# lrm2017/Fastest_Image_Pattern_Matching

Hardware: AMD Instinct MI355X
Metric: template matches/sec + ms/search, 4024×3036 src ±180°; HBM GB/s vs roofline (higher is better)
Workload: dtype u8

## Files before the change

fastest_image_pattern_matching_amd/csrc/fpm_kernels.hip:

```cpp
#include <float.h>
#include <stdio.h>
#include <stdlib.h>
#include <limits.h>

#include <map>
#include <mutex>
#include <type_traits>
#include <utility>

#include "../../include/fpm.h"
#include "fpm_kernels.h"
#include "fpm_model.h"
#include "fpm_rrect.h"

static void ensure_lds_attr(const void* fn, size_t bytes) {
    if (bytes <= 65536) return;
    int dev = 0;
    (void)hipGetDevice(&dev);
    static std::mutex mu;
    static std::map<std::pair<int, const void*>, size_t> done;
    std::lock_guard<std::mutex> lock(mu);
    size_t& cur = done[std::make_pair(dev, fn)];
    if (bytes <= cur) return;
    (void)hipFuncSetAttribute(fn, hipFuncAttributeMaxDynamicSharedMemorySize, (int)bytes);
// ... 2191 lines not shown

__device__ __forceinline__ int mad24(int a, int b, int c) {
    int d;
    asm("v_mad_i32_i24 %0, %1, %2, %3" : "=v"(d) : "v"(a), "v"(b), "v"(c));
    return d;
}

__device__ __forceinline__ int ft_tap_interior(const uint8_t* FT, int off, int ftw, int X, int Y) {
    const uint32_t fx = X & (kInterTab - 1), fy = Y & (kInterTab - 1);
    const uint32_t* F = (const uint32_t*)FT;
    const int off1 = off + ftw;
    const uint32_t* q0 = F + (off >> 2);
    const uint32_t* q1 = F + (off1 >> 2);
    const uint32_t r0 = __builtin_amdgcn_alignbyte(q0[1], q0[0], (uint32_t)off);
    const uint32_t r1 = __builtin_amdgcn_alignbyte(q1[1], q1[0], (uint32_t)off1);
    const uint32_t wx = 32u + fx * 255u;
    const uint32_t h0 = __builtin_amdgcn_udot4(r0, wx, 0u, false), h1 = __builtin_amdgcn_udot4(r1, wx, 0u, false);
    return (int)((__umul24(32u - fy, h0) + __umul24(fy, h1) + 512u) >> 10);
}

__device__ __forceinline__ int ft_tap_bytes(const uint8_t* FT, int off, int ftw, int X, int Y) {
    const int fx = X & (kInterTab - 1), fy = Y & (kInterTab - 1);
    const uint8_t* p = FT + off;
    const int v0 = p[0], v1 = p[1], v2 = p[ftw], v3 = p[ftw + 1];
    const int h0 = 32 * v0 + __mul24(fx, v1 - v0), h1 = 32 * v2 + __mul24(fx, v3 - v2);
    return (32 * h0 + __mul24(fy, h1 - h0) + 512) >> 10;
}

typedef __attribute__((address_space(3))) const uint8_t fpm_lds_u8;
__device__ __forceinline__ uint32_t lds_offset_of(const uint8_t* p) { return (uint32_t)(size_t)(fpm_lds_u8*)p; }
__device__ __forceinline__ void lds_taps(uint32_t off, int ftw, int v[4]) {
    fpm_lds_u8* p = (fpm_lds_u8*)(size_t)off;
    fpm_lds_u8* q = (fpm_lds_u8*)(size_t)(off + ftw);
    v[0] = p[0]; v[1] = p[1]; v[2] = q[0]; v[3] = q[1];
}
__device__ __forceinline__ int bilerp24(const int v[4], int fx, int fy) {
    const int h0 = mad24(fx, v[1] - v[0], v[0] << 5), h1 = mad24(fx, v[3] - v[2], v[2] << 5);
    return mad24(fy, h1 - h0, (h0 << 5) + 512) >> 10;
}
typedef unsigned short fpm_u16x2v __attribute__((ext_vector_type(2)));
__device__ __forceinline__ uint32_t bilerp_row4(const int v[4][4], const int fx[4], const int fy[4]) {
    uint32_t r[4];
#pragma unroll
    for (int u = 0; u < 4; ++u) {
        const uint32_t a02 = __builtin_amdgcn_perm((uint32_t)v[u][2], (uint32_t)v[u][0], 0x0c040c00u);
        const uint32_t a13 = __builtin_amdgcn_perm((uint32_t)v[u][3], (uint32_t)v[u][1], 0x0c040c00u);
        const fpm_u16x2v d = __builtin_bit_cast(fpm_u16x2v, a13) - __builtin_bit_cast(fpm_u16x2v, a02);
        const fpm_u16x2v b = __builtin_bit_cast(fpm_u16x2v, a02) << (fpm_u16x2v)5;
        uint32_t h;
        asm("v_pk_mad_u16 %0, %1, %2, %3 op_sel_hi:[0,1,1]"
            : "=v"(h) : "v"(fx[u]), "v"(__builtin_bit_cast(uint32_t, d)), "v"(__builtin_bit_cast(uint32_t, b)));
        const uint32_t wy = (uint32_t)mad24(fy[u], 64 * 0x10000 - 64, 64 * 32);
        r[u] = __builtin_amdgcn_udot2(__builtin_bit_cast(fpm_u16x2v, h), __builtin_bit_cast(fpm_u16x2v, wy), 64u * 512u,
                                      false);
    }
    return __builtin_amdgcn_perm(r[1], r[0], 0x0c0c0602u) | __builtin_amdgcn_perm(r[3], r[2], 0x06020c0cu);
}
template <int PITCH>
__device__ __forceinline__ void lds_taps16(const uint32_t off[4], int v[4][4]) {
    asm volatile("ds_read_u8 %0, %16\n\tds_read_u8 %1, %16 offset:1\n\tds_read_u8 %2, %16 offset:%20\n\t"
                 "ds_read_u8 %3, %16 offset:%21\n\t"
                 "ds_read_u8 %4, %17\n\tds_read_u8 %5, %17 offset:1\n\tds_read_u8 %6, %17 offset:%20\n\t"
                 "ds_read_u8 %7, %17 offset:%21\n\t"
                 "ds_read_u8 %8, %18\n\tds_read_u8 %9, %18 offset:1\n\tds_read_u8 %10, %18 offset:%20\n\t"
                 "ds_read_u8 %11, %18 offset:%21\n\t"
                 "ds_read_u8 %12, %19\n\tds_read_u8 %13, %19 offset:1\n\tds_read_u8 %14, %19 offset:%20\n\t"
                 "ds_read_u8 %15, %19 offset:%21\n\t"
                 "s_waitcnt lgkmcnt(0)"
                 : "=&v"(v[0][0]), "=&v"(v[0][1]), "=&v"(v[0][2]), "=&v"(v[0][3]), "=&v"(v[1][0]), "=&v"(v[1][1]),
                   "=&v"(v[1][2]), "=&v"(v[1][3]), "=&v"(v[2][0]), "=&v"(v[2][1]), "=&v"(v[2][2]), "=&v"(v[2][3]),
                   "=&v"(v[3][0]), "=&v"(v[3][1]), "=&v"(v[3][2]), "=&v"(v[3][3])
                 : "v"(off[0]), "v"(off[1]), "v"(off[2]), "v"(off[3]), "i"(PITCH), "i"(PITCH + 1)
                 : "memory");
}

__device__ __forceinline__ int ft_tap_general(const uint8_t* FT, int ftw, int bxa, int by0, int W, int H, int X, int Y) {
    const int sx = sat_s16(X >> kInterBits), sy = sat_s16(Y >> kInterBits);
    const int fx = X & (kInterTab - 1), fy = Y & (kInterTab - 1);
    const uint8_t* p = FT + (sy - by0) * ftw + (sx - bxa);
    int v0, v1, v2, v3;
    if ((unsigned)sx < (unsigned)(W - 1) && (unsigned)sy < (unsigned)(H - 1)) {
        v0 = p[0]; v1 = p[1]; v2 = p[ftw]; v3 = p[ftw + 1];
    } else if (sx >= W || sx + 1 < 0 || sy >= H || sy + 1 < 0) {
        return 0;
    } else {
        const bool x0 = sx >= 0 && sx < W, x1 = sx + 1 >= 0 && sx + 1 < W;
        const bool y0 = sy >= 0 && sy < H, y1 = sy + 1 >= 0 && sy + 1 < H;
        v0 = x0 && y0 ? p[0] : 0;
        v1 = x1 && y0 ? p[1] : 0;
        v2 = x0 && y1 ? p[ftw] : 0;
        v3 = x1 && y1 ? p[ftw + 1] : 0;
    }
    const int h0 = 32 * v0 + fx * (v1 - v0), h1 = 32 * v2 + fx * (v3 - v2);
    return (32 * h0 + fy * (h1 - h0) + 512) >> 10;
}

__device__ __forceinline__ int roi_base(const RoiArgs& a) { return a.slot_base; }
__device__ __forceinline__ void roi_slot(const RoiArgs& a, int slot, int& id, int& jj) {
    const int ri = roi_base(a) + slot;
    const int li = ri / a.n3;
    jj = ri - li * a.n3;
    id = a.live[li];
}

__device__ __forceinline__ int roi_count(const RoiArgs& a) {
    int rois = *a.live_count * a.n3 - roi_base(a);
    return rois < 0 ? 0 : (rois > a.slot_cap ? a.slot_cap : rois);
}

__device__ __forceinline__ void wave_sync() {
    __builtin_amdgcn_fence(__ATOMIC_RELEASE, "wavefront");
    __builtin_amdgcn_wave_barrier();
    __builtin_amdgcn_fence(__ATOMIC_ACQUIRE, "wavefront");
}

template <int B>
__device__ __forceinline__ void stage_footprint(uint8_t* FT, int ftw, int wpr, int fth, const uint8_t* gsrc,
                                                size_t gpitch, int gx0, int gP, int lane) {
    const int c = lane & 15;
    if (c >= wpr) return;
    const int gx = gx0 + 4 * c;
    const bool inb = gx < gP;
    const uint8_t* gp = gsrc + 4 * c + (size_t)(lane >> 4) * gpitch;
    uint8_t* lp = FT + 4 * c + (lane >> 4) * ftw;
    const size_t gstep = 4 * gpitch;
    const int lstep = 4 * ftw;
    for (int r0 = lane >> 4; r0 < fth; r0 += 4 * B) {
        uint32_t v[B];
#pragma unroll
        for (int i = 0; i < B; ++i) v[i] = (inb && r0 + 4 * i < fth) ? *(const uint32_t*)(gp + i * gstep) : 0u;
#pragma unroll
        for (int i = 0; i < B; ++i)
            if (r0 + 4 * i < fth) *(uint32_t*)(lp + i * lstep) = v[i];
        gp += B * gstep;
        lp += B * lstep;
    }
}
typedef __attribute__((address_space(3))) void* fpm_lds_vp;
typedef __attribute__((address_space(1))) void* fpm_gbl_vp;
__device__ __forceinline__ void stage_footprint_dma(uint8_t* FT, int wpr, int fth, const uint8_t* gsrc,
                                                    size_t gpitch, int lane) {
    const int total = wpr * fth;
    int r = lane / wpr, c = lane - r * wpr;
    const int dr = 64 / wpr, dc = 64 - dr * wpr;
    for (int i0 = 0; i0 < total; i0 += 64) {
        if (i0 + lane < total)
            __builtin_amdgcn_global_load_lds((fpm_gbl_vp)(gsrc + (size_t)r * gpitch + 4 * c), (fpm_lds_vp)(FT + 4 * i0), 4, 0, 0);
        r += dr;
        c += dc;
        if (c >= wpr) { c -= wpr; ++r; }
    }
    asm volatile("s_waitcnt vmcnt(0)" ::: "memory");
}
__device__ __forceinline__ void stage_block16(uint8_t* dst, int dp, const uint8_t* src, size_t sp, int rows, int q16,
                                              int tid, int nthr) {
    const int total = rows * q16;
    int r = tid / q16, c = tid - (tid / q16) * q16;
    const int dr = nthr / q16, dc = nthr - dr * q16;
    for (int i0 = tid; i0 < total; i0 += 4 * nthr) {
        uint4 v[4];
        int rr[4], cc[4];
#pragma unroll
        for (int k = 0; k < 4; ++k) {
            rr[k] = r; cc[k] = c;
            v[k] = (i0 + k * nthr < total) ? *(const uint4*)(src + (size_t)r * sp + 16 * c) : make_uint4(0, 0, 0, 0);
            r += dr; c += dc;
            if (c >= q16) { c -= q16; ++r; }
        }
#pragma unroll
        for (int k = 0; k < 4; ++k)
            if (i0 + k * nthr < total) *(uint4*)(dst + (size_t)rr[k] * dp + 16 * cc[k]) = v[k];
    }
}
__device__ __forceinline__ void stage_block4(uint8_t* dst, int dp, const uint8_t* src, size_t sp, int rows, int wpr,
                                             int gx0, int gP, int tid, int nthr) {
    const int total = rows * wpr;
    int r = tid / wpr, c = tid - (tid / wpr) * wpr;
    const int dr = nthr / wpr, dc = nthr - dr * wpr;
    for (int i0 = tid; i0 < total; i0 += 8 * nthr) {
        uint32_t v[8];
        int rr[8], cc[8];
#pragma unroll
        for (int k = 0; k < 8; ++k) {
            rr[k] = r; cc[k] = c;
            v[k] = (i0 + k * nthr < total && gx0 + 4 * c < gP) ? *(const uint32_t*)(src + (size_t)r * sp + 4 * c) : 0u;
            r += dr; c += dc;
            if (c >= wpr) { c -= wpr; ++r; }
        }
#pragma unroll
        for (int k = 0; k < 8; ++k)
            if (i0 + k * nthr < total) *(uint32_t*)(dst + (size_t)rr[k] * dp + 4 * cc[k]) = v[k];
    }
}

constexpr int kPatchTw = 64, kPatchTh = 16;
constexpr int kPatchFtPitch = 76;
constexpr int kPatchFtRows = 72;

constexpr int kPatchTabWords = 2 * kPatchTw + 2 * kPatchTh;
constexpr int kPatchFtBytes = kPatchFtPitch * kPatchFtRows + 16;

struct PatchTile {
    int job;
    int x0, y0;
    int bxa, by0;
    bool in_lds;
    const uint8_t* img;
};

__device__ __forceinline__ PatchTile patch_tile_stage_at(const PatchArgs& a, int32_t* tab, uint8_t* FT, int tid, int p,
                                                         int tx, int ty) {
    int32_t* const ad = tab;
    int32_t* const bd = tab + kPatchTw;
    int32_t* const X0 = tab + 2 * kPatchTw;
    int32_t* const Y0 = X0 + kPatchTh;
    const int x0 = tx * kPatchTw, y0 = ty * kPatchTh;
    const PatchJob& j = a.jobs[p];
    if (tid < kPatchTw) {
        const int x = x0 + tid;
        ad[tid] = rint_i(j.M[0] * x * kAbScale);
        bd[tid] = rint_i(j.M[3] * x * kAbScale);
    } else if (tid < kPatchTw + kPatchTh) {
        const int y = y0 + tid - kPatchTw;
        X0[tid - kPatchTw] = rint_i((j.M[1] * y + j.M[2]) * kAbScale) + kRoundDelta;
        Y0[tid - kPatchTw] = rint_i((j.M[4] * y + j.M[5]) * kAbScale) + kRoundDelta;
    }
    __syncthreads();
    const int cx = (a.pw - x0 < kPatchTw ? a.pw - x0 : kPatchTw) - 1, cy = (a.ph - y0 < kPatchTh ? a.ph - y0 : kPatchTh) - 1;
    int bx0 = INT_MAX, bx1 = INT_MIN, by0 = INT_MAX, by1 = INT_MIN;
#pragma unroll
    for (int k = 0; k < 4; ++k) {
        const int c = (k & 1) ? cx : 0, r = (k & 2) ? cy : 0;
        const int sx = (X0[r] + ad[c]) >> kAbBits, sy = (Y0[r] + bd[c]) >> kAbBits;
        bx0 = sx < bx0 ? sx : bx0; bx1 = sx > bx1 ? sx : bx1;
        by0 = sy < by0 ? sy : by0; by1 = sy > by1 ? sy : by1;
    }
    bx0 -= 1; by0 -= 1; bx1 += 2; by1 += 2;
    const int bxa = bx0 & ~3;
    const int wpr = ((bx1 - bxa) >> 2) + 1;
    const int fth = by1 - by0 + 1;
    const bool fits = bx0 >= 0 && by0 >= 0 && bx1 < a.sw && by1 < a.sh && a.sw <= 32768 && a.sh <= 32768 &&
                      wpr <= kPatchFtPitch / 4 && fth <= kPatchFtRows;
    const bool in_lds = __builtin_amdgcn_readfirstlane((int)fits) != 0;
    const uint8_t* img = a.level0 + (size_t)j.src * a.img_stride;
    if (in_lds) {
        stage_block4(FT, kPatchFtPitch, img + (size_t)by0 * a.sp + bxa, (size_t)a.sp, fth, wpr, bxa, a.sp, tid, 256);
        __syncthreads();
    }
    return {p, x0, y0, bxa, by0, in_lds, img};
}

__device__ __forceinline__ PatchTile patch_tile_stage(const PatchArgs& a, int32_t* tab, uint8_t* FT, int tid) {
    const int b = xcd_remap(blockIdx.x, gridDim.x);
    const int tiles = a.tiles_x * a.tiles_y;
    const int p = b / tiles, t = b - p * tiles;
    const int ty = t / a.tiles_x, tx = t - ty * a.tiles_x;
    return patch_tile_stage_at(a, tab, FT, tid, p, tx, ty);
}

__device__ __forceinline__ uint32_t patch_sample4(const PatchArgs& a, const PatchTile& T, const int32_t* tab,
                                                  const uint8_t* FT, int r, int gx, int nu) {
    const int Xr = tab[2 * kPatchTw + r], Yr = tab[2 * kPatchTw + kPatchTh + r];
    const int4 A = *(const int4*)(tab + gx), B = *(const int4*)(tab + kPatchTw + gx);
    const int av[4] = {A.x, A.y, A.z, A.w}, bv[4] = {B.x, B.y, B.z, B.w};
    uint32_t word = 0;
#pragma unroll
    for (int u = 0; u < 4; ++u) {
        if (u >= nu) break;
        const int X = (Xr + av[u]) >> (kAbBits - kInterBits), Y = (Yr + bv[u]) >> (kAbBits - kInterBits);
        int v;
        if (T.in_lds)
            v = ft_tap_bytes(FT, ((Y >> kInterBits) - T.by0) * kPatchFtPitch + (X >> kInterBits) - T.bxa, kPatchFtPitch, X, Y);
        else
            v = warp_tap(T.img, a.sw, a.sh, a.sp, X, Y, 0);
        word |= (uint32_t)v << (8 * u);
    }
    return word;
}

__device__ __forceinline__ void patch_store4(uint8_t* d, uint32_t word, int nu, bool dword) {
    if (dword && nu == 4) {
        *(uint32_t*)d = word;
    } else {
        for (int u = 0; u < nu; ++u) d[u] = (uint8_t)(word >> (8 * u));
    }
}

__global__ __launch_bounds__(256) void k_patch_warp(const PatchArgs a) {
    __shared__ __attribute__((aligned(16))) int32_t tab[kPatchTabWords];
    __shared__ __attribute__((aligned(16))) uint8_t FT[kPatchFtBytes];
    const int tid = threadIdx.x;
    const PatchTile T = patch_tile_stage(a, tab, FT, tid);
    const int r = tid >> 4, gx = (tid & 15) * 4;
    const int x = T.x0 + gx, y = T.y0 + r;
    if (x >= a.pw || y >= a.ph) return;
    const int nu = a.pw - x < 4 ? a.pw - x : 4;
    const uint32_t word = patch_sample4(a, T, tab, FT, r, gx, nu);
    patch_store4(a.out + a.jobs[T.job].out_off + (size_t)y * a.row_stride + x, word, nu, a.dword != 0);
}

template <int CTRL, int ROWS, bool MAX>
__device__ __forceinline__ uint32_t dpp_fold(uint32_t v) {
    const uint32_t o = (uint32_t)__builtin_amdgcn_update_dpp(0, (int)v, CTRL, ROWS, 0xf, false);
    return MAX ? (o > v ? o : v) : v + o;
}
template <bool MAX>
__device__ __forceinline__ uint32_t wave_fold(uint32_t v) {
    v = dpp_fold<0xb1, 0xf, MAX>(v);
    v = dpp_fold<0x4e, 0xf, MAX>(v);
    v = dpp_fold<0x141, 0xf, MAX>(v);
    v = dpp_fold<0x140, 0xf, MAX>(v);
    v = dpp_fold<0x142, 0xa, MAX>(v);
    v = dpp_fold<0x143, 0xc, MAX>(v);
    return (uint32_t)__builtin_amdgcn_readlane((int)v, 63);
}

__device__ __forceinline__ void vote_box(unsigned long long mk, int u, int& cnt, int& cmin, int& cmax, int& rmin,
                                         int& rmax) {
    if (mk == 0) return;
    cnt += __popcll(mk);
    const uint32_t cols = (uint32_t)(mk | (mk >> 16) | (mk >> 32) | (mk >> 48)) & 0xffffu;
    const int lo = 4 * (__ffs(cols) - 1) + u, hi = 4 * (31 - __clz(cols)) + u;
    cmin = lo < cmin ? lo : cmin; cmax = hi > cmax ? hi : cmax;
    const int rlo = (__ffsll(mk) - 1) >> 4, rhi = (63 - __clzll(mk)) >> 4;
    rmin = rlo < rmin ? rlo : rmin; rmax = rhi > rmax ? rhi : rmax;
}
// ... 1803 lines not shown
            const uint32_t l0 = row[0] ^ 0x80808080u, l1 = row[1] ^ 0x80808080u;
            const int wr = tw >> 2;
            const uint32_t x0 = row[wr], x1 = row[wr + 1], x2 = row[wr + 2];
            const uint32_t e0 = __builtin_amdgcn_alignbyte(x1, x0, (uint32_t)tw) ^ 0x80808080u;
            const uint32_t e1 = __builtin_amdgcn_alignbyte(x2, x1, (uint32_t)tw) ^ 0x80808080u;
            s1 += (uint32_t)__builtin_amdgcn_mov_dpp((int)s1, 0xB1, 0xF, 0xF, false);
            s2 += (uint32_t)__builtin_amdgcn_mov_dpp((int)s2, 0xB1, 0xF, 0xF, false);
            s1 += (uint32_t)__builtin_amdgcn_mov_dpp((int)s1, 0x4E, 0xF, 0xF, false);
            s2 += (uint32_t)__builtin_amdgcn_mov_dpp((int)s2, 0x4E, 0xF, 0xF, false);
#pragma unroll
            for (int h = 0; h < 2; ++h) {
                const int dx = qq + 4 * h;
                if (dx < 7) {
                    const uint32_t ml0 = dx >= 4 ? 0xffffffffu : (1u << (8 * dx)) - 1u;
                    const uint32_t ml1 = dx <= 4 ? 0u : (1u << (8 * (dx - 4))) - 1u;
                    const uint32_t mr0 = dx >= 4 ? 0u : ~((1u << (8 * dx)) - 1u);
                    const uint32_t mr1 = dx <= 4 ? 0xffffu : dx == 5 ? 0xff00u : 0u;
                    const uint32_t a0 = l0 & ml0, a1 = l1 & ml1, b0 = e0 & mr0, b1 = e1 & mr1;
                    uint32_t q1 = __builtin_amdgcn_udot4(a0, 0x01010101u, 0u, false);
                    q1 = __builtin_amdgcn_udot4(a1, 0x01010101u, q1, false);
                    q1 = __builtin_amdgcn_udot4(b0, 0x01010101u, q1, false);
                    q1 = __builtin_amdgcn_udot4(b1, 0x01010101u, q1, false);
                    uint32_t q2 = __builtin_amdgcn_udot4(a0, a0, 0u, false);
                    q2 = __builtin_amdgcn_udot4(a1, a1, q2, false);
                    q2 = __builtin_amdgcn_udot4(b0, b0, q2, false);
                    q2 = __builtin_amdgcn_udot4(b1, b1, q2, false);
                    const uint32_t v1 = s1 - q1, v2 = s2 - q2;
                    wi[r * 7 + dx] = v1;
                    wq[r * 7 + dx] = v2;
                    if (MODE != 6) {
                        if (r < rb) { u1[h] = v1; u2[h] = v2; }
                        const uint32_t eo = (uint32_t)slot * (uint32_t)kRoiEdgeWords;
                        if (band == 0 && r < 6) {
                            const uint32_t o = eo + (uint32_t)(r * 7 + dx);
                            a.wedge[o] = v1;
                            a.wedge[o + 84u] = v2;
                        }
                        if (band == nband - 1 && r >= rb) {
                            const uint32_t o = eo + (uint32_t)((6 + r - rb) * 7 + dx);
                            a.wedge[o] = v1;
                            a.wedge[o + 84u] = v2;
                        }
                    }
                }
            }
        }
        if (RS == 1 && MODE != 7 && MODE != 6 && wv < 2) {
#pragma unroll
            for (int h = 0; h < 2; ++h) {
                uint32_t r1 = u1[h], lo = u2[h] & 0xffffu, hi = u2[h] >> 16;
#pragma unroll
                for (int m = 4; m <= 32; m <<= 1) {
                    r1 += (uint32_t)__shfl_xor((int)r1, m, 64);
                    lo += (uint32_t)__shfl_xor((int)lo, m, 64);
                    hi += (uint32_t)__shfl_xor((int)hi, m, 64);
                }
                if (lane < 4 && lane + 4 * h < 7) {
                    bt1[8 * wv + lane + 4 * h] = r1;
                    bt2[8 * wv + lane + 4 * h] = (uint64_t)lo + ((uint64_t)hi << 16);
                }
            }
        }
        __syncthreads();
        auto band_totals = [&]() {
            if (MODE == 6 || MODE == 7 || tid < 128 || tid >= 128 + 7) return;
            uint32_t dx = (uint32_t)(tid - 128);
            asm volatile("" : "+v"(dx));
            const bool two = rb > kMmaRows;
            const uint32_t s1 = bt1[dx] + (two ? bt1[8 + dx] : 0u);
            const uint64_t s2 = bt2[dx] + (two ? bt2[8 + dx] : 0ull);
            const uint32_t wo = ((uint32_t)slot * (uint32_t)nband + (uint32_t)band) * 7u + dx;
            a.wtot[wo] = s1;
            a.wtotq[wo] = s2;
        };
        const bool active = kMmaRows * mt < rb && kMmaRows * nt < nsrc;
        if (FPM_CORR_PRIO == 1) __builtin_amdgcn_s_setprio(1);
        if (MODE != 2 && active) {
            int sr = kMmaRows * nt + n;
            if (sr >= nsrc) sr = 0;
            const uint8_t* bp = SB + (size_t)sr * SBp + 16 * g;
            fpm_v4i acc[7];
            if (FPM_CORR_PRIO == 2) __builtin_amdgcn_s_setprio(1);
            if (NK > 0)
                band_mfma_regs<NA>(Areg, bp, a.nk, acc);
            else
                band_mfma_ga(a.tmpl8 + (size_t)(T0 + kMmaRows * mt + n) * a.tp8 + 16 * g, bp, a.nk, acc);
            if (FPM_CORR_PRIO == 2) __builtin_amdgcn_s_setprio(0);
            uint32_t* rs_out = a.rowsum + (((size_t)th * 49 + 3) & ~(size_t)3) * slot + (size_t)T0 * 49;
            const uint32_t kFix = 16384u * (uint32_t)tw;
            int t0 = kMmaRows * mt + 4 * g;
            asm volatile("" : "+v"(t0));
            const int s_ = kMmaRows * nt + n;
            const uint4 ts4 = *(const uint4*)(lts + t0);
#pragma unroll
            for (int r = 0; r < 4; ++r) {
                const int t = t0 + r, dy = s_ - t;
                if (t < rb && s_ < nsrc && dy >= 0 && dy < 7) {
                    const uint32_t ts = r == 0 ? ts4.x : r == 1 ? ts4.y : r == 2 ? ts4.z : ts4.w;
                    if (MODE == 5) {
                        uint32_t x = ts;
#pragma unroll
                        for (int d = 0; d < 7; ++d) x += (uint32_t)acc[d][r];
                        if (x == 0x9e3779b9u && a.W < 0) rs_out[t] = x;
                        continue;
                    }
                    const uint32_t o = (uint32_t)(t * 49 + dy * 7);
                    if (SE) {
#pragma unroll
                        for (int d = 0; d < 7; ++d) rsb[o + d] = (uint32_t)acc[d][r] + 128u * (wi[s_ * 7 + d] + ts) - kFix;
                        continue;
                    }
#pragma unroll
                    for (int d = 0; d < 7; ++d) rs_out[o + d] = (uint32_t)acc[d][r] + 128u * (wi[s_ * 7 + d] + ts) - kFix;
                }
            }
        }
        if (FPM_CORR_PRIO == 1) __builtin_amdgcn_s_setprio(0);
        band_totals();
        if (SE) { pv_slot = slot; pv_T0 = T0; pv_rb = rb; }
    }
    if (SE && pv_slot >= 0) {
        __syncthreads();
        flush();
    }
}

__device__ __forceinline__ CandState cand_step_state(CandState s, int n3, const AngleNode* nodes, double thr, int W,
                                                     int H, int mark_reached0, const float* score, const int* mx,
                                                     const int* my, const AngleNode* next_nodes = nullptr,
                                                     int jj = 0, AngleNode* next_nd = nullptr, int nnext = 1) {
    int imax = 0;
    double big = -1;
    for (int k = 0; k < n3; ++k)
        if ((double)score[k] > big) { imax = k; big = score[k]; }
    if ((double)score[imax] < thr) {
        s.alive = 0;
        return s;
    }
    const int child = s.node * n3 + imax;
    const AngleNode nd = nodes[child];
    if (next_nodes)
        for (int k = 0; k < nnext; ++k) next_nd[k] = next_nodes[child * n3 + jj + k];
    const F2 sc = f2((W - 1) / 2.0f, (H - 1) / 2.0f);
    const F2 r0 = rotate_pt(f2(s.lt.x * 2, s.lt.y * 2), sc, nd.c, nd.s);
    const F2 pad = f2(r0.x - 3, r0.y - 3);
    F2 p = f2((float)((double)mx[imax] + pad.x), (float)((double)my[imax] + pad.y));
    p = rotate_pt(p, sc, nd.cn, nd.sn);
    s.lt = p;
    s.node = child;
    s.reached0 = mark_reached0;
    return s;
}

struct SmallLayout {
    int sbp, tbp, rh, u, tab, sum, rs, sc, ts, total;
};
__host__ __device__ inline int isqrt_ceil(int n) {
    int d = 0;
    while ((d + 1) * (d + 1) <= n) ++d;
    return d * d == n ? d : d + 1;
}
__host__ __device__ inline int small_footprint_bound(int rw, int rh) {
    const int d = isqrt_ceil((rw - 1) * (rw - 1) + (rh - 1) * (rh - 1)) + 2;
    return ((d + 16) * (d + 6) + 15) & ~15;
}
__host__ __device__ inline SmallLayout small_layout(int tw, int th, int nw = 4) {
    SmallLayout L;
    L.sbp = roi_pitch_calc(tw);
    L.tbp = tmpl_lds_pitch(64 * ((tw + 63) / 64));
    L.rh = th + 6;
    const int th16 = (th + kMmaRows - 1) / kMmaRows * kMmaRows;
    L.u = ((L.rh + 16) * L.sbp + 15) & ~15;
    const int fb = small_footprint_bound(tw + 6, th + 6);
    const int fp = fb < nw * ROI_FT ? fb : nw * ROI_FT;
    const int ub = th16 * L.tbp > fp ? th16 * L.tbp : fp;
    L.tab = L.u + ub;
    L.sum = L.tab + 4 * (2 * L.sbp + 2 * ((L.rh + 3) & ~3));
    const int rs_size = 4 * kBandRows * 49;
    const int after_sums = L.sum + 4 * (2 * L.rh + 2 * 7 * L.rh) + 8 * 49 * 2;
    if (th16 * L.tbp + rs_size <= L.sum - L.u) {
        L.rs = L.u + th16 * L.tbp;
        L.sc = after_sums;
    } else {
        L.rs = after_sums;
        L.sc = L.rs + rs_size;
    }
    L.ts = L.sc + 4 * 64;
    L.total = L.ts + 4 * th16;
    return L;
}
constexpr int kSmallLdsMax = 72 * 1024;
bool roi_small_fits(int tw, int th) { return th <= 256 && small_layout(tw, th).total <= kSmallLdsMax; }
size_t roi_small_lds(int tw, int th) { return (size_t)small_layout(tw, th).total; }

template <int MODE, int WPE = 3, bool PROL = false, int NT = 256>
__global__ __launch_bounds__(NT) __attribute__((amdgpu_waves_per_eu(WPE))) void k_roi_small(RoiArgs a) {
    constexpr int NW = NT / 64;
    extern __shared__ __attribute__((aligned(16))) uint8_t smem[];
    const int tw = a.tw, th = a.th, RW = tw + 6, RH = th + 6, W = a.W, H = a.H;
    const SmallLayout LY = small_layout(tw, th, NW);
    const int SBp = LY.sbp, TBp = LY.tbp;
    uint8_t* SB = smem;
    uint8_t* TB = smem + LY.u;
    uint8_t* FTall = smem + LY.u;
    int32_t* lad = (int32_t*)(smem + LY.tab);
    int32_t* lbd = lad + SBp;
    int32_t* lx0 = lbd + SBp;
    int32_t* ly0 = lx0 + ((RH + 3) & ~3);
    uint32_t* rall = (uint32_t*)(smem + LY.sum);
    uint32_t* rallq = rall + RH;
    uint32_t* wi = rallq + RH;
    uint32_t* wq = wi + RH * 7;
    uint64_t* tot = (uint64_t*)(((uintptr_t)(wq + RH * 7) + 7) & ~(uintptr_t)7);
    uint32_t* rs = (uint32_t*)(smem + LY.rs);
    float* sc = (float*)(smem + LY.sc);
    uint32_t* lts = (uint32_t*)(smem + LY.ts);
    const int tid = threadIdx.x, lane = tid & 63, wv = tid >> 6;
    const int rois = roi_count(a);
    const int q4 = SBp >> 4, nwr = (RW + 3) >> 2;
    const int txn = (RW + ROI_T - 1) / ROI_T, tyn = (RH + ROI_T - 1) / ROI_T;
    const int g = lane >> 4, n = lane & 15;
    const int lr = lane >> 3, lg = lane & 7;
    auto STAMP = [&](int k) {
        if (MODE == 9 && tid == 0 && blockIdx.x < 64) a.stamps[blockIdx.x * 16 + k] = __builtin_readcyclecounter();
    };
    for (int slot = blockIdx.x; slot < rois; slot += gridDim.x) {
        STAMP(0);
        int id, jj;
        roi_slot(a, slot, id, jj);
        const uint8_t* lvl = a.level + (size_t)(id / a.per_source) * a.level_stride;
        CandState st = a.state[id];
        AngleNode nd;
        if (PROL) {
            if (st.alive) {
                const RoiRecord* r = a.prev_rec + (size_t)id * a.n3;
                float score[3];
                int mx[3], my[3];
                for (int k = 0; k < a.n3; ++k) { score[k] = r[k].score; mx[k] = r[k].mx; my[k] = r[k].my; }
                st = cand_step_state(st, a.n3, a.prev_nodes, a.prev_thr, a.prev_W, a.prev_H, 0, score, mx, my, a.nodes,
                                     jj, &nd);
                if (jj == 0 && tid == 0 && st.alive) atomicAdd(a.live_out_count, 1);
            }
            if (jj == 0 && tid == 0) a.state_out[id] = st;
            if (!st.alive) continue;
        } else {
            nd = a.nodes[st.node * a.n3 + jj];
        }
        __syncthreads();
        {
            double M[6];
            roi_matrix(W, H, f2(st.lt.x * 2, st.lt.y * 2), nd.c, nd.s, M);
            for (int x = tid; x < RW; x += NT) {
                lad[x] = rint_i(M[0] * x * kAbScale);
                lbd[x] = rint_i(M[3] * x * kAbScale);
            }
            for (int y = tid; y < RH; y += NT) {
                lx0[y] = rint_i((M[1] * y + M[2]) * kAbScale) + kRoundDelta;
                ly0[y] = rint_i((M[4] * y + M[5]) * kAbScale) + kRoundDelta;
            }
        }
        __syncthreads();
        STAMP(1);
        int gbx0 = INT_MAX, gbx1 = INT_MIN, gby0 = INT_MAX, gby1 = INT_MIN;
#pragma unroll
        for (int k = 0; k < 4; ++k) {
            const int c = (k & 1) ? RW - 1 : 0, r = (k & 2) ? RH - 1 : 0;
            const int X = (lx0[r] + lad[c]) >> (kAbBits - kInterBits);
            const int Y = (ly0[r] + lbd[c]) >> (kAbBits - kInterBits);
            gbx0 = min(gbx0, X >> kInterBits); gbx1 = max(gbx1, X >> kInterBits);
            gby0 = min(gby0, Y >> kInterBits); gby1 = max(gby1, Y >> kInterBits);
        }
        const bool g_interior = gbx0 - 1 >= 0 && gbx1 + 1 <= W - 2 && gby0 - 1 >= 0 && gby1 + 1 <= H - 2;
        gbx0 = max(gbx0 - 1, 0); gby0 = max(gby0 - 1, 0);
        gbx1 = min(gbx1 + 2, W - 1); gby1 = min(gby1 + 2, H - 1);
        const bool g_any = gbx0 <= gbx1 && gby0 <= gby1;
        const int gbxa = gbx0 & ~3;
        const int gftw = g_any ? ((gbx1 - gbxa + 4) & ~3) + 4 : 4;
        const int gfth = g_any ? gby1 - gby0 + 1 : 0;
        const int gobase = gby0 * gftw + gbxa;
        if (g_any && gftw * gfth <= LY.tab - LY.u) {
            uint8_t* FT = FTall;
            const int wpr = gftw >> 2;
            stage_block4(FT, gftw, lvl + (size_t)gby0 * a.P + gbxa, a.P, gfth, wpr, gbxa, a.P, tid, NT);
            __syncthreads();
            STAMP(8);
            const int ngrp = (RW + 3) >> 2;
            const int nrl = NT / ngrp;
            const int rl = tid / ngrp, c0 = 4 * (tid - rl * ngrp);
            int ad4[4], bd4[4];
#pragma unroll
            for (int u = 0; u < 4; ++u) { ad4[u] = lad[c0 + u]; bd4[u] = lbd[c0 + u]; }
            if (g_interior && MODE != 5) {
                const int xo = ((int)lds_offset_of(FT) - gbxa) << kAbBits, yo = -(gby0 << kAbBits);
                const int nvalid = RW - c0;
                const uint32_t colmask = nvalid >= 4 ? 0xffffffffu : (nvalid <= 0 ? 0u : (1u << (8 * nvalid)) - 1u);
                for (int r = rl < nrl ? rl : RH; r < RH; r += nrl) {
                    const int x0r = lx0[r] + xo, y0r = ly0[r] + yo;
                    uint32_t off[4];
                    int fxv[4], fyv[4], v[4][4];
#pragma unroll
                    for (int u = 0; u < 4; ++u) {
                        const int sxv = x0r + ad4[u], syv = y0r + bd4[u];
                        fxv[u] = __builtin_amdgcn_ubfe(sxv, kAbBits - kInterBits, kInterBits);
                        fyv[u] = __builtin_amdgcn_ubfe(syv, kAbBits - kInterBits, kInterBits);
                        off[u] = (uint32_t)mad24(syv >> kAbBits, gftw, sxv >> kAbBits);
                    }
#pragma unroll
                    for (int u = 0; u < 4; ++u) lds_taps(off[u], gftw, v[u]);
                    uint32_t pk = 0;
#pragma unroll
                    for (int u = 0; u < 4; ++u) pk |= (uint32_t)bilerp24(v[u], fxv[u], fyv[u]) << (8 * u);
                    *(uint32_t*)(SB + r * SBp + c0) = pk & colmask;
                }
            } else {
                for (int r = rl < nrl ? rl : RH; r < RH; r += nrl) {
                    const int X0 = lx0[r], Y0 = ly0[r];
                    uint32_t pk = 0;
#pragma unroll
                    for (int u = 0; u < 4; ++u) {
                        const int X = (X0 + ad4[u]) >> (kAbBits - kInterBits);
                        const int Y = (Y0 + bd4[u]) >> (kAbBits - kInterBits);
                        int v;
                        if (g_interior) {
                            const int off = mad24(Y >> kInterBits, gftw, (X >> kInterBits) - gobase);
                            v = ft_tap_bytes(FT, off, gftw, X, Y);
                        } else {
                            v = ft_tap_general(FT, gftw, gbxa, gby0, W, H, X, Y);
                        }
                        if (c0 + u >= RW) v = 0;
                        pk |= (uint32_t)v << (8 * u);
                    }
                    *(uint32_t*)(SB + r * SBp + c0) = pk;
                }
            }
            STAMP(9);
        } else if (!g_any) {
            for (int i = tid; i < RH * (SBp >> 2); i += NT) ((uint32_t*)SB)[i] = 0u;
        } else {
            const bool tile_bufs = NW * ROI_FT <= LY.tab - LY.u;
            uint8_t* FT = FTall + wv * ROI_FT;
            for (int task = wv; task < txn * tyn; task += NW) {
                const int ty = task / txn, tx = task - ty * txn;
                const int cx0 = tx * ROI_T, cx1 = min(cx0 + ROI_T, RW) - 1;
                const int ry0 = ty * ROI_T, ry1 = min(ry0 + ROI_T, RH) - 1;
                int bx0 = INT_MAX, bx1 = INT_MIN, by0 = INT_MAX, by1 = INT_MIN;
#pragma unroll
                for (int k = 0; k < 4; ++k) {
                    const int c = (k & 1) ? cx1 : cx0, r = (k & 2) ? ry1 : ry0;
                    const int X = (lx0[r] + lad[c]) >> (kAbBits - kInterBits);
                    const int Y = (ly0[r] + lbd[c]) >> (kAbBits - kInterBits);
                    bx0 = min(bx0, X >> kInterBits); bx1 = max(bx1, X >> kInterBits);
                    by0 = min(by0, Y >> kInterBits); by1 = max(by1, Y >> kInterBits);
                }
                const bool interior = bx0 - 1 >= 0 && bx1 + 1 <= W - 2 && by0 - 1 >= 0 && by1 + 1 <= H - 2;
                bx0 = max(bx0 - 1, 0); by0 = max(by0 - 1, 0);
                bx1 = min(bx1 + 2, W - 1); by1 = min(by1 + 2, H - 1);
                const bool any = bx0 <= bx1 && by0 <= by1;
                const int bxa = bx0 & ~3;
                int ftw = any ? ((bx1 - bxa + 4) & ~3) : 0;
                if (((ftw >> 2) & 1) == 0) ftw += 4;
                const int fth = any ? by1 - by0 + 1 : 0;
                const int wpr = ftw >> 2;
                const bool in_lds = tile_bufs && wpr <= 16 && ftw * fth <= ROI_FT;
                wave_sync();
                if (any && in_lds) stage_footprint<4>(FT, ftw, wpr, fth, lvl + (size_t)by0 * a.P + bxa, a.P, bxa, a.P, lane);
                wave_sync();
                const int c0 = cx0 + 4 * lg;
                if (c0 > cx1) continue;
                for (int i = 0; i < 4; ++i) {
                    const int r = ry0 + lr + 8 * i;
                    if (r > ry1) break;
                    const int X0 = lx0[r], Y0 = ly0[r];
                    uint32_t pk = 0;
#pragma unroll
                    for (int u = 0; u < 4; ++u) {
                        const int X = (X0 + lad[c0 + u]) >> (kAbBits - kInterBits);
                        const int Y = (Y0 + lbd[c0 + u]) >> (kAbBits - kInterBits);
                        int v;
                        if (interior && in_lds) {
                            const int off = mad24(Y >> kInterBits, ftw, (X >> kInterBits) - (by0 * ftw + bxa));
                            v = MODE == 5 ? ft_tap_bytes(FT, off, ftw, X, Y) : ft_tap_interior(FT, off, ftw, X, Y);
                        } else {
                            v = in_lds ? ft_tap_general(FT, ftw, bxa, by0, W, H, X, Y) : roi_tap(lvl, W, H, a.P, X, Y);
                        }
                        if (c0 + u >= RW) v = 0;
                        pk |= (uint32_t)v << (8 * u);
                    }
                    *(uint32_t*)(SB + r * SBp + c0) = pk;
                }
            }
        }
        __syncthreads();
        if (MODE == 1) continue;
        STAMP(2);
        for (int r = tid; r < RH; r += NT) {
            const uint32_t* row = (const uint32_t*)(SB + (size_t)r * SBp);
            uint32_t s1 = 0, s2 = 0;
            int k = 0;
            for (; k + 8 <= nwr; k += 8) {
                uint32_t x[8];
#pragma unroll
                for (int u = 0; u < 8; ++u) x[u] = row[k + u];
#pragma unroll
                for (int u = 0; u < 8; ++u) {
                    s1 = __builtin_amdgcn_udot4(x[u], 0x01010101u, s1, false);
                    s2 = __builtin_amdgcn_udot4(x[u], x[u], s2, false);
                }
            }
            for (; k < nwr; ++k) {
                const uint32_t x = row[k];
                s1 = __builtin_amdgcn_udot4(x, 0x01010101u, s1, false);
                s2 = __builtin_amdgcn_udot4(x, x, s2, false);
            }
            rall[r] = s1;
            rallq[r] = s2;
        }
        __syncthreads();
        for (int i = tid; i < RH * q4; i += NT) {
            uint4* v = (uint4*)SB + i;
            uint4 x = *v;
            x.x ^= 0x80808080u; x.y ^= 0x80808080u; x.z ^= 0x80808080u; x.w ^= 0x80808080u;
            *v = x;
        }
        {
            const int trows = (th + kMmaRows - 1) / kMmaRows * kMmaRows;
            stage_block16(TB, TBp, (const uint8_t*)a.tmpl8, a.tp8, trows, a.tp8 >> 4, tid, NT);
            if (WPE < 4)
                for (int i = tid; i < (NT >= 256 ? min(trows, NT) : trows); i += NT) lts[i] = (uint32_t)a.tsum[i];
        }
        __syncthreads();
        STAMP(3);
        for (int r = tid; r < RH; r += NT) {
            const uint8_t* sbr = SB + (size_t)r * SBp;
            uint32_t lv[6], rv[6];
#pragma unroll
            for (int c = 0; c < 6; ++c) { lv[c] = sbr[c] ^ 0x80u; rv[c] = sbr[tw + c] ^ 0x80u; }
            uint32_t q1 = rall[r], q2 = rallq[r];
#pragma unroll
            for (int c = 0; c < 6; ++c) { q1 -= rv[c]; q2 -= rv[c] * rv[c]; }
#pragma unroll
            for (int dx = 0; dx < 7; ++dx) {
                if (dx > 0) {
                    q1 += rv[dx - 1] - lv[dx - 1];
                    q2 += rv[dx - 1] * rv[dx - 1] - lv[dx - 1] * lv[dx - 1];
                }
                wi[r * 7 + dx] = q1;
                wq[r * 7 + dx] = q2;
            }
        }
        if (tid < 98) tot[tid] = 0;
        __syncthreads();
        STAMP(4);
#pragma unroll 1
        for (int q = tid; q < (NT >= 4 * 49 ? (tid < 4 * 49 ? tid + 1 : 0) : 4 * 49); q += NT) {
            const int part = q / 49, k = q - part * 49, pdy = k / 7, ddx = k - pdy * 7;
            const int t0 = part * th / 4, t1 = (part + 1) * th / 4;
            uint64_t s1 = 0, s2 = 0;
            int t = t0;
            for (; t + 8 <= t1; t += 8) {
                uint32_t x[8], y[8];
#pragma unroll
                for (int u = 0; u < 8; ++u) { x[u] = wi[(t + u + pdy) * 7 + ddx]; y[u] = wq[(t + u + pdy) * 7 + ddx]; }
#pragma unroll
                for (int u = 0; u < 8; ++u) { s1 += x[u]; s2 += y[u]; }
            }
            for (; t < t1; ++t) { s1 += wi[(t + pdy) * 7 + ddx]; s2 += wq[(t + pdy) * 7 + ddx]; }
            atomicAdd((unsigned long long*)&tot[k], (unsigned long long)s1);
            atomicAdd((unsigned long long*)&tot[49 + k], (unsigned long long)s2);
        }
        if (MODE == 2) continue;
        STAMP(5);
        float accF = 0.f;
        uint64_t accI = 0;
        const uint32_t kFix = 16384u * (uint32_t)tw;
        for (int T0 = 0; T0 < th; T0 += kBandRows) {
            const int rb = min(kBandRows, th - T0), nsrc = rb + 6;
#pragma unroll
            for (int pass = 0; pass < (4 + NW - 1) / NW; ++pass) {
            const int p = wv + pass * NW, mt = p & 1, nt = mt + (p >> 1);
            if (p < 4 && kMmaRows * mt < rb && kMmaRows * nt < nsrc) {
                const uint8_t* ap = TB + (size_t)(T0 + kMmaRows * mt + n) * TBp + 16 * g;
                const uint8_t* bp = SB + (size_t)(T0 + kMmaRows * nt + n) * SBp + 16 * g;
                fpm_v4i acc[7];
                band_mfma(ap, bp, a.nk, acc);
                const int s_ = kMmaRows * nt + n;
#pragma unroll
                for (int r = 0; r < 4; ++r) {
                    const int t = kMmaRows * mt + 4 * g + r, dy = s_ - t;
                    if (t < rb && s_ < nsrc && dy >= 0 && dy < 7) {
                        const uint32_t ts = WPE < 4 ? lts[T0 + t] : (uint32_t)a.tsum[T0 + t];
#pragma unroll
                        for (int d = 0; d < 7; ++d)
                            rs[t * 49 + dy * 7 + d] = (uint32_t)acc[d][r] + 128u * (wi[(T0 + s_) * 7 + d] + ts) - kFix;
                    }
                }
            }
            }
            __syncthreads();
            if (MODE != 3 && tid < 49) {
                if (a.fold) {
                    int t = 0;
                    for (; t + 8 <= rb; t += 8) {
                        uint32_t x[8];
#pragma unroll
                        for (int u = 0; u < 8; ++u) x[u] = rs[(t + u) * 49 + tid];
#pragma unroll
                        for (int u = 0; u < 8; ++u) accF = accF + (float)(int)x[u];
                    }
                    for (; t < rb; ++t) accF = accF + (float)(int)rs[t * 49 + tid];
                } else {
                    for (int t = 0; t < rb; ++t) accI += rs[t * 49 + tid];
                }
            }
            __syncthreads();
        }
        if (tid < 49) {
            const double num = a.fold ? (double)accF : (double)(float)(double)accI;
            sc[tid] = ccoeff(num, (double)tot[tid], (double)tot[49 + tid], a.mean, a.norm, a.inv_area);
        }
        __syncthreads();
        STAMP(6);
        if (wv == 0) {
            float v = lane < 49 ? sc[lane] : -INFINITY;
            int bi = lane < 49 ? lane : 64;
            if (v != v) { v = -INFINITY; bi = 64 + lane; }
            wave_better_reduce(v, bi);
            const float s0 = sc[0];
            if (s0 != s0 || bi >= 64) bi = 0;
            const float best = sc[bi];
            const int mx = bi % 7, my = bi / 7;
            RoiRecord r;
            r.score = best;
            r.mx = (int16_t)mx;
            r.my = (int16_t)my;
            const int border = (mx == 0 || my == 0 || mx == 6 || my == 6) ? 1 : 0;
            r.on_border = border;
            for (int x = -1; x <= 1; ++x)
                for (int y = -1; y <= 1; ++y) r.vec[(x + 1) * 3 + (y + 1)] = border ? 0.f : sc[(my + y) * 7 + (mx + x)];
            if (lane == 0) a.rec[(size_t)id * a.n3 + jj] = r;
        }
        STAMP(7);
    }
}

__device__ int cand_step_one(const RoiArgs& a, int id, const float* score, const int* mx, const int* my,
                             CandState* so = nullptr, AngleNode* nn = nullptr) {
    CandState* out = a.state_out ? a.state_out : a.state;
    CandState s = a.state[id];
    if (!s.alive) {
        out[id] = s;
        return -1;
    }
    s = cand_step_state(s, a.n3, a.nodes, a.thr, a.W, a.H, a.mark_reached0, score, mx, my, nn ? a.nt_nodes : nullptr,
                        0, nn, a.n3);
    out[id] = s;
    if (so) *so = s;
    if (!s.alive) return -1;
    const int p = atomicAdd(a.live_out_count, 1);
    a.live_out[p] = id;
    return p;
}

__device__ __forceinline__ void cand_next_tables(const RoiArgs& a, int id, int p, const CandState& s,
                                                 const AngleNode& nd, int j, int lane) {
    roi_tables_fill(a.nt_tab, a.tdesc, a.tdesc_stride, a.nt_tabw, a.nt_tabh, a.nt_tw, a.nt_th, a.nt_W, a.nt_H,
                    p * a.n3 + j, s.lt, nd, (id / a.per_source) << kTileSrcShift, lane, 64);
}

__global__ __launch_bounds__(256) void k_cand_step(RoiArgs a) {
    const int n = *a.live_count;
    for (int li = blockIdx.x * 256 + threadIdx.x; li < n; li += gridDim.x * 256) {
        const int id = a.live[li];
        const RoiRecord* r = a.rec + (size_t)id * a.n3;
        float score[3];
        int mx[3], my[3];
        for (int k = 0; k < a.n3; ++k) { score[k] = r[k].score; mx[k] = r[k].mx; my[k] = r[k].my; }
        cand_step_one(a, id, score, mx, my);
    }
}

__global__ __launch_bounds__(192) void k_cand_step_tab(RoiArgs a) {
    __shared__ int pos;
    __shared__ CandState ns;
    __shared__ AngleNode nn[3];
    const int n = *a.live_count;
    const int lane = threadIdx.x & 63, j = threadIdx.x >> 6;
    for (int li = blockIdx.x; li < n; li += gridDim.x) {
        const int id = a.live[li];
        __syncthreads();
        if (threadIdx.x == 0) {
            const RoiRecord* r = a.rec + (size_t)id * a.n3;
            float score[3];
            int mx[3], my[3];
            for (int k = 0; k < a.n3; ++k) { score[k] = r[k].score; mx[k] = r[k].mx; my[k] = r[k].my; }
            CandState s;
            pos = cand_step_one(a, id, score, mx, my, &s, a.nt_tab ? nn : nullptr);
            ns = s;
        }
        __syncthreads();
        if (pos >= 0 && j < a.n3) cand_next_tables(a, id, pos, ns, nn[j], j, lane);
    }
}

template <int ROWS>
struct EvalBlk {
    static_assert(ROWS * 49 % 4 == 0, "a block is whole uint4 of the [th][49] series");
    static constexpr int dma = (ROWS * 49 / 4 + 63) / 64;
    static constexpr int buf = dma * 1024;
};

template <int ROWS>
__device__ void eval_roi(const RoiArgs& a, int slot, int lane, uint8_t* blk, float* sc, RoiRecord* out,
                         RoiRecord* keep) {
    constexpr int kEvalRows = ROWS, kEvalDma = EvalBlk<ROWS>::dma, kEvalBuf = EvalBlk<ROWS>::buf;
    const int th = a.th;
    if (a.equal1) {
        if (lane == 0) {
            RoiRecord r;
            r.score = 1.f; r.mx = 0; r.my = 0; r.on_border = 1;
            for (int k = 0; k < 9; ++k) r.vec[k] = 0.f;
            *out = r;
// ... 808 lines not shown
```

Baseline: 37230.

## Fuse ROI window-sum statistics into one pass with DMA template staging

The 0x80 sign flip now happens when the source ROI is written, which removes the separate XOR pass over the buffer. Row sums, the 7-wide sliding window sums and per-column totals are computed in a single pass, with four lanes per row combined through DPP reductions. The 49-offset totals are then derived from the column totals by adding and subtracting head and tail rows, instead of re-summing every row. Template staging switches to asynchronous global_load_lds DMA that overlaps with the statistics work, which saves two barriers and several LDS passes at the cost of inline assembly that manipulates m0 and depends on correct waitcnt ordering.

```diff
diff --git a/fastest_image_pattern_matching_amd/csrc/fpm_kernels.hip b/fastest_image_pattern_matching_amd/csrc/fpm_kernels.hip
--- a/fastest_image_pattern_matching_amd/csrc/fpm_kernels.hip
+++ b/fastest_image_pattern_matching_amd/csrc/fpm_kernels.hip
@@ -2367,26 +2367,6 @@
     }
     asm volatile("s_waitcnt vmcnt(0)" ::: "memory");
 }
-__device__ __forceinline__ void stage_block16(uint8_t* dst, int dp, const uint8_t* src, size_t sp, int rows, int q16,
-                                              int tid, int nthr) {
-    const int total = rows * q16;
-    int r = tid / q16, c = tid - (tid / q16) * q16;
-    const int dr = nthr / q16, dc = nthr - dr * q16;
-    for (int i0 = tid; i0 < total; i0 += 4 * nthr) {
-        uint4 v[4];
-        int rr[4], cc[4];
-#pragma unroll
-        for (int k = 0; k < 4; ++k) {
-            rr[k] = r; cc[k] = c;
-            v[k] = (i0 + k * nthr < total) ? *(const uint4*)(src + (size_t)r * sp + 16 * c) : make_uint4(0, 0, 0, 0);
-            r += dr; c += dc;
-            if (c >= q16) { c -= q16; ++r; }
-        }
-#pragma unroll
-        for (int k = 0; k < 4; ++k)
-            if (i0 + k * nthr < total) *(uint4*)(dst + (size_t)rr[k] * dp + 16 * cc[k]) = v[k];
-    }
-}
 __device__ __forceinline__ void stage_block4(uint8_t* dst, int dp, const uint8_t* src, size_t sp, int rows, int wpr,
                                              int gx0, int gP, int tid, int nthr) {
     const int total = rows * wpr;
@@ -4496,6 +4476,15 @@
     return s;
 }
 
+constexpr uint32_t kFlip4 = 0x80808080u;
+__device__ __forceinline__ uint32_t quad_lane_fold(uint32_t v) {
+    v += (uint32_t)__builtin_amdgcn_mov_dpp((int)v, 0x124, 0xF, 0xF, false);
+    v += (uint32_t)__builtin_amdgcn_mov_dpp((int)v, 0x128, 0xF, 0xF, false);
+    v += (uint32_t)__shfl_xor((int)v, 16, 64);
+    v += (uint32_t)__shfl_xor((int)v, 32, 64);
+    return v;
+}
+
 struct SmallLayout {
     int sbp, tbp, rh, u, tab, sum, rs, sc, ts, total;
 };
@@ -4551,17 +4540,16 @@
     int32_t* lbd = lad + SBp;
     int32_t* lx0 = lbd + SBp;
     int32_t* ly0 = lx0 + ((RH + 3) & ~3);
-    uint32_t* rall = (uint32_t*)(smem + LY.sum);
-    uint32_t* rallq = rall + RH;
-    uint32_t* wi = rallq + RH;
+    uint32_t* wi = (uint32_t*)(smem + LY.sum) + 2 * RH;
     uint32_t* wq = wi + RH * 7;
     uint64_t* tot = (uint64_t*)(((uintptr_t)(wq + RH * 7) + 7) & ~(uintptr_t)7);
     uint32_t* rs = (uint32_t*)(smem + LY.rs);
     float* sc = (float*)(smem + LY.sc);
+    uint64_t* colT = (uint64_t*)(smem + LY.sc);
     uint32_t* lts = (uint32_t*)(smem + LY.ts);
     const int tid = threadIdx.x, lane = tid & 63, wv = tid >> 6;
     const int rois = roi_count(a);
-    const int q4 = SBp >> 4, nwr = (RW + 3) >> 2;
+    const int nwr = (RW + 3) >> 2;
     const int txn = (RW + ROI_T - 1) / ROI_T, tyn = (RH + ROI_T - 1) / ROI_T;
     const int g = lane >> 4, n = lane & 15;
     const int lr = lane >> 3, lg = lane & 7;
@@ -4591,6 +4579,8 @@
             nd = a.nodes[st.node * a.n3 + jj];
         }
         __syncthreads();
+        STAMP(11);
+        if (tid < 14) colT[tid] = 0;
         {
             double M[6];
             roi_matrix(W, H, f2(st.lt.x * 2, st.lt.y * 2), nd.c, nd.s, M);
@@ -4654,7 +4644,7 @@
                     uint32_t pk = 0;
 #pragma unroll
                     for (int u = 0; u < 4; ++u) pk |= (uint32_t)bilerp24(v[u], fxv[u], fyv[u]) << (8 * u);
-                    *(uint32_t*)(SB + r * SBp + c0) = pk & colmask;
+                    *(uint32_t*)(SB + r * SBp + c0) = (pk & colmask) ^ kFlip4;
                 }
             } else {
                 for (int r = rl < nrl ? rl : RH; r < RH; r += nrl) {
@@ -4674,12 +4664,12 @@
                         if (c0 + u >= RW) v = 0;
                         pk |= (uint32_t)v << (8 * u);
                     }
-                    *(uint32_t*)(SB + r * SBp + c0) = pk;
+                    *(uint32_t*)(SB + r * SBp + c0) = pk ^ kFlip4;
                 }
             }
             STAMP(9);
         } else if (!g_any) {
-            for (int i = tid; i < RH * (SBp >> 2); i += NT) ((uint32_t*)SB)[i] = 0u;
+            for (int i = tid; i < RH * (SBp >> 2); i += NT) ((uint32_t*)SB)[i] = kFlip4;
         } else {
             const bool tile_bufs = NW * ROI_FT <= LY.tab - LY.u;
             uint8_t* FT = FTall + wv * ROI_FT;
@@ -4730,87 +4720,111 @@
                         if (c0 + u >= RW) v = 0;
                         pk |= (uint32_t)v << (8 * u);
                     }
-                    *(uint32_t*)(SB + r * SBp + c0) = pk;
+                    *(uint32_t*)(SB + r * SBp + c0) = pk ^ kFlip4;
                 }
             }
         }
         __syncthreads();
         if (MODE == 1) continue;
         STAMP(2);
-        for (int r = tid; r < RH; r += NT) {
-            const uint32_t* row = (const uint32_t*)(SB + (size_t)r * SBp);
-            uint32_t s1 = 0, s2 = 0;
-            int k = 0;
-            for (; k + 8 <= nwr; k += 8) {
-                uint32_t x[8];
-#pragma unroll
-                for (int u = 0; u < 8; ++u) x[u] = row[k + u];
-#pragma unroll
-                for (int u = 0; u < 8; ++u) {
-                    s1 = __builtin_amdgcn_udot4(x[u], 0x01010101u, s1, false);
-                    s2 = __builtin_amdgcn_udot4(x[u], x[u], s2, false);
-                }
-            }
-            for (; k < nwr; ++k) {
-                const uint32_t x = row[k];
-                s1 = __builtin_amdgcn_udot4(x, 0x01010101u, s1, false);
-                s2 = __builtin_amdgcn_udot4(x, x, s2, false);
-            }
-            rall[r] = s1;
-            rallq[r] = s2;
-        }
-        __syncthreads();
-        for (int i = tid; i < RH * q4; i += NT) {
-            uint4* v = (uint4*)SB + i;
-            uint4 x = *v;
-            x.x ^= 0x80808080u; x.y ^= 0x80808080u; x.z ^= 0x80808080u; x.w ^= 0x80808080u;
-            *v = x;
-        }
+        const int trows = (th + kMmaRows - 1) / kMmaRows * kMmaRows;
         {
-            const int trows = (th + kMmaRows - 1) / kMmaRows * kMmaRows;
-            stage_block16(TB, TBp, (const uint8_t*)a.tmpl8, a.tp8, trows, a.tp8 >> 4, tid, NT);
-            if (WPE < 4)
-                for (int i = tid; i < (NT >= 256 ? min(trows, NT) : trows); i += NT) lts[i] = (uint32_t)a.tsum[i];
-        }
-        __syncthreads();
-        STAMP(3);
-        for (int r = tid; r < RH; r += NT) {
-            const uint8_t* sbr = SB + (size_t)r * SBp;
-            uint32_t lv[6], rv[6];
-#pragma unroll
-            for (int c = 0; c < 6; ++c) { lv[c] = sbr[c] ^ 0x80u; rv[c] = sbr[tw + c] ^ 0x80u; }
-            uint32_t q1 = rall[r], q2 = rallq[r];
-#pragma unroll
-            for (int c = 0; c < 6; ++c) { q1 -= rv[c]; q2 -= rv[c] * rv[c]; }
-#pragma unroll
-            for (int dx = 0; dx < 7; ++dx) {
-                if (dx > 0) {
-                    q1 += rv[dx - 1] - lv[dx - 1];
-                    q2 += rv[dx - 1] * rv[dx - 1] - lv[dx - 1] * lv[dx - 1];
-                }
-                wi[r * 7 + dx] = q1;
-                wq[r * 7 + dx] = q2;
-            }
-        }
-        if (tid < 98) tot[tid] = 0;
+            const int tq16 = a.tp8 >> 4, tq = TBp >> 4, units = trows * tq;
+            const uint32_t qinv = 0xffffffffu / (uint32_t)tq + 1u;
+            const int wvu = __builtin_amdgcn_readfirstlane(wv);
+            for (int u0 = 64 * wvu; u0 < units; u0 += 64 * NW) {
+                const int i = u0 + lane;
+                if (i < units) {
+                    const int r = (int)__umulhi((uint32_t)i, qinv), c = min(i - r * tq, tq16 - 1);
+                    const uint8_t* gp = (const uint8_t*)a.tmpl8 + (size_t)r * a.tp8 + 16 * c;
+                    const uint32_t ldsa = __builtin_amdgcn_readfirstlane(lds_offset_of(TB) + 16u * (uint32_t)u0);
+                    uint32_t keep;
+                    asm volatile("s_mov_b32 %0, m0\n\ts_mov_b32 m0, %2\n\ts_nop 0\n\tglobal_load_lds_dwordx4 %1, off\n\t"
+                                 "s_mov_b32 m0, %0"
+                                 : "=&s"(keep) : "v"(gp), "s"(ldsa) : "memory");
+                }
+            }
+        }
+        {
+            int tq = tid;
+            asm volatile("" : "+v"(tq));
+            const int sub = tq & 3;
+            uint32_t c1[2] = {0, 0};
+            uint64_t c2[2] = {0, 0};
+            for (int r = tq >> 2; r < RH; r += NT / 4) {
+                const uint8_t* sbr = SB + (size_t)r * SBp;
+                const uint32_t* row = (const uint32_t*)sbr;
+                uint32_t s1 = 0, s2 = 0;
+                int k = sub;
+                for (; k + 12 < nwr; k += 16) {
+                    uint32_t x[4];
+#pragma unroll
+                    for (int u = 0; u < 4; ++u) x[u] = row[k + 4 * u] ^ kFlip4;
+#pragma unroll
+                    for (int u = 0; u < 4; ++u) {
+                        s1 = __builtin_amdgcn_udot4(x[u], 0x01010101u, s1, false);
+                        s2 = __builtin_amdgcn_udot4(x[u], x[u], s2, false);
+                    }
+                }
+                for (; k < nwr; k += 4) {
+                    const uint32_t x = row[k] ^ kFlip4;
+                    s1 = __builtin_amdgcn_udot4(x, 0x01010101u, s1, false);
+                    s2 = __builtin_amdgcn_udot4(x, x, s2, false);
+                }
+                uint32_t lv[6], rv[6];
+#pragma unroll
+                for (int c = 0; c < 6; ++c) { lv[c] = sbr[c] ^ 0x80u; rv[c] = sbr[tw + c] ^ 0x80u; }
+                s1 += (uint32_t)__builtin_amdgcn_mov_dpp((int)s1, 0xB1, 0xF, 0xF, false);
+                s2 += (uint32_t)__builtin_amdgcn_mov_dpp((int)s2, 0xB1, 0xF, 0xF, false);
+                s1 += (uint32_t)__builtin_amdgcn_mov_dpp((int)s1, 0x4E, 0xF, 0xF, false);
+                s2 += (uint32_t)__builtin_amdgcn_mov_dpp((int)s2, 0x4E, 0xF, 0xF, false);
+                uint32_t q1 = s1, q2 = s2;
+#pragma unroll
+                for (int c = 0; c < 6; ++c) { q1 -= rv[c]; q2 -= rv[c] * rv[c]; }
+#pragma unroll
+                for (int dx = 0; dx < 7; ++dx) {
+                    if (dx > 0) {
+                        q1 += rv[dx - 1] - lv[dx - 1];
+                        q2 += rv[dx - 1] * rv[dx - 1] - lv[dx - 1] * lv[dx - 1];
+                    }
+                    if ((dx & 3) == sub) {
+                        wi[r * 7 + dx] = q1;
+                        wq[r * 7 + dx] = q2;
+                        if (r < th) { c1[dx >> 2] += q1; c2[dx >> 2] += q2; }
+                    }
+                }
+            }
+#pragma unroll
+            for (int h = 0; h < 2; ++h) {
+                const uint32_t t1 = quad_lane_fold(c1[h]);
+                const uint32_t lo = quad_lane_fold((uint32_t)c2[h] & 0xffffffu), hi = quad_lane_fold((uint32_t)(c2[h] >> 24));
+                const int cl = (tq & 63) + 4 * h;
+                if ((tq & 63) < 4 && cl < 7) {
+                    atomicAdd((unsigned long long*)&colT[cl], (unsigned long long)t1);
+                    atomicAdd((unsigned long long*)&colT[7 + cl], (unsigned long long)lo + ((unsigned long long)hi << 24));
+                }
+            }
+        }
+        if (WPE < 4)
+            for (int i = tid; i < (NT >= 256 ? min(trows, NT) : trows); i += NT) lts[i] = (uint32_t)a.tsum[i];
+        asm volatile("s_waitcnt vmcnt(0)" ::: "memory");
         __syncthreads();
         STAMP(4);
-#pragma unroll 1
-        for (int q = tid; q < (NT >= 4 * 49 ? (tid < 4 * 49 ? tid + 1 : 0) : 4 * 49); q += NT) {
-            const int part = q / 49, k = q - part * 49, pdy = k / 7, ddx = k - pdy * 7;
-            const int t0 = part * th / 4, t1 = (part + 1) * th / 4;
-            uint64_t s1 = 0, s2 = 0;
-            int t = t0;
-            for (; t + 8 <= t1; t += 8) {
-                uint32_t x[8], y[8];
-#pragma unroll
-                for (int u = 0; u < 8; ++u) { x[u] = wi[(t + u + pdy) * 7 + ddx]; y[u] = wq[(t + u + pdy) * 7 + ddx]; }
-#pragma unroll
-                for (int u = 0; u < 8; ++u) { s1 += x[u]; s2 += y[u]; }
-            }
-            for (; t < t1; ++t) { s1 += wi[(t + pdy) * 7 + ddx]; s2 += wq[(t + pdy) * 7 + ddx]; }
-            atomicAdd((unsigned long long*)&tot[k], (unsigned long long)s1);
-            atomicAdd((unsigned long long*)&tot[49 + k], (unsigned long long)s2);
+        int ta = tid;
+        asm volatile("" : "+v"(ta));
+        if (ta < 98) {
+            const int stat = ta >= 49 ? 1 : 0, k = ta - 49 * stat, pdy = k / 7, ddx = k - pdy * 7;
+            const uint32_t* w = stat ? wq : wi;
+            uint32_t hd[6], tl[6];
+#pragma unroll
+            for (int r = 0; r < 6; ++r) {
+                hd[r] = r < pdy ? w[r * 7 + ddx] : 0u;
+                tl[r] = r < pdy ? w[(th + r) * 7 + ddx] : 0u;
+            }
+            uint64_t v = colT[7 * stat + ddx];
+#pragma unroll
+            for (int r = 0; r < 6; ++r) v = v + tl[r] - hd[r];
+            tot[ta] = v;
         }
         if (MODE == 2) continue;
         STAMP(5);
```

Measured after the change: 37400 (median of 6 runs). About the same (+0.5%).
